# nanoporetech/taiyaki

Measured on AMD Instinct MI355X. Metric: signal-chunks/sec (T=4000) flip-flop train step, higher is better.
Workload: dtype f32; 1 GPU; configs[1]: mLstm_flipflop r9.4.1 DNA, chunk_len=4000 (T=800 blocks), 128 chunks/GPU, size 256, HIP flip-flop CRF loss + logZ, gradient maxima/clipping, AdamW; config_id=2, model=mLstm_flipflop, global_batch=128, chunk_len=4000, launch=hipGraph replay of forward+loss and of AdamW, eager backward, hw_queues=4, conv=gemm, lstm=miopen, batches=pre-assembled, cycled from HBM, parallelism=dp1 (reads sharded; one flat RCCL gradient all-reduce after backward)

## Files before the change

### taiyaki_amd/csrc/lstm_kernels.hip

```cpp
#include "dispatch.h"
#include "ff_common.h"
#include "lstm_bwd_layout.h"
#include "lstm_fwd_layout.h"
#include "rnn_common.h"

namespace tk {
namespace {

template <int U>
constexpr int threads_for() { return U == 48 ? 384 : U <= 32 ? 256 : 512; }
template <int H, int U>
constexpr int bwd_threads_for() { return U == 48 ? 2 * H : threads_for<U>(); }

template <int M>
__device__ __forceinline__ float xor_lane(float v) {
    static_assert(M == 1 || M == 2 || M == 4, "a partner inside the lane's group of 8");
    const int x = __float_as_int(v);
    if constexpr (M == 1) {
        return __int_as_float(__builtin_amdgcn_update_dpp(0, x, 0xB1, 0xF, 0xF, true));
    } else if constexpr (M == 2) {
        return __int_as_float(__builtin_amdgcn_update_dpp(0, x, 0x4E, 0xF, 0xF, true));
    } else {
        const int y = __builtin_amdgcn_update_dpp(0, x, 0x141, 0xF, 0xF, true);
        return __int_as_float(__builtin_amdgcn_update_dpp(0, y, 0x1B, 0xF, 0xF, true));
    }
}

template <int M, int RQ, int NA>
__device__ __forceinline__ void halve_rounds(float (&acc)[NA], int rq) {
    if constexpr (M < RQ) {
        constexpr int n = NA / (2 * M);
        const bool up = (rq & M) != 0;
#pragma unroll
        for (int a = 0; a < n; ++a) {
            const float send = up ? acc[a] : acc[a + n];
            const float keep = up ? acc[a + n] : acc[a];
            acc[a] = keep + xor_lane<M>(send);
        }
        halve_rounds<2 * M, RQ>(acc, rq);
    }
}

template <int H, int C, int U, bool VL, bool SAVE>
__device__ __forceinline__ void lstm_fwd_lanes_body(const float *__restrict__ gx, const float *__restrict__ whh, int T,
                                                    Cols cols, int reverse, int ngroups, float *__restrict__ y,
                                                    float *__restrict__ gates, float *__restrict__ cell, u64 *hbuf,
                                                    uint32_t *status, const int32_t *__restrict__ lengths) {
    constexpr int NT = threads_for<U>();
    const int N = cols.n, LD = cols.ld();
    constexpr int G = H / U;
    constexpr LstmFwdLanes FL(NT, H, U, C);
    constexpr int KP = FL.KP, KS = FL.KS, PR = FL.PR, CK = FL.CK;
    constexpr int NG = H * C / NT;
    static_assert(FL.ok() && KP == 8 && NG * NT == H * C && FL.gate_lane_xor(1) == 4 && FL.gate_lane_xor(2) == 2 &&
                      FL.gate_lane_xor(3) == 6,
                  "whole rows in 16-byte reads; the partial sums and the four gates of a column inside 8 lanes of a wave");
    constexpr int U4 = U / 4;
    constexpr int NQ = SAVE ? (6 * C * U4 + NT - 1) / NT : 1;
    static_assert(U % 4 == 0, "a row of the staging block is whole 16-byte chunks");
    __shared__ __attribute__((aligned(16))) float hs[2][H * C];
    __shared__ __attribute__((aligned(16))) float stg[SAVE ? 2 : 1][SAVE ? 6 * C * U : 4];
    __shared__ int give_up;

    int group, member;
    place(G, group, member);
    const int tid = threadIdx.x;
    const int j0 = member * U, n0 = group * C;
    const int u = tid / KP, kp = tid % KP;

    float w[4][KS];
#pragma unroll
    for (int g = 0; g < 4; ++g)
#pragma unroll
        for (int i = 0; i < KS; ++i) w[g][i] = whh[((size_t)g * H + j0 + u) * H + FL.k(kp, i)];
    settle(w);

    const int gate = FL.gate(kp), col = FL.col(kp, 0);
    const bool cell_lane = gate == 0;
    const int n = n0 + col;
    bool fetch[CK], valid[CK];
    float cst[CK], held[CK];
    int len[CK];
#pragma unroll
    for (int v = 0; v < CK; ++v) {
        fetch[v] = n + v < N;
        valid[v] = cell_lane && fetch[v];
        cst[v] = held[v] = 0.f;
        len[v] = 0;
        if constexpr (VL) len[v] = !valid[v] ? 0 : lengths ? lengths[n + v] : T;
    }

    for (int i = tid; i < H * C; i += NT) hs[0][i] = 0.f;
    if (tid == 0) give_up = 0;

    const size_t H4 = 4 * (size_t)H;
    float *rp[NQ];
    size_t rpitch[NQ];
    if constexpr (SAVE) {
#pragma unroll
        for (int i = 0; i < NQ; ++i) {
            const int q = tid + i * NT, row = q / U4, v = row / C, nn = n0 + row % C;
            const size_t w = v < 2 ? (size_t)H : H4;
            float *base = v == 0 ? y : v == 1 ? cell : gates + (size_t)(v - 2) * H;
            rpitch[i] = (size_t)LD * w;
            rp[i] = q < 6 * C * U4 && nn < N ? base + (size_t)nn * w + j0 + 4 * (q % U4) : nullptr;
        }
    }
    const float *gx0 = gx + (size_t)n * H4 + (size_t)gate * H + j0 + u;
    float gq[CK];
#pragma unroll
    for (int v = 0; v < CK; ++v) gq[v] = fetch[v] ? gx0[(size_t)(reverse ? T - 1 : 0) * LD * H4 + v * H4] : 0.f;
    __syncthreads();

    for (int s = 0; s < T; ++s) {
        const int t = reverse ? T - 1 - s : s;
        float *hb = hs[s & 1];
        settle(gq);
        if (s > 0) {
            const u64 *src = hbuf + ((size_t)((s - 1) & 1) * ngroups + group) * (H * C);
            float v[NG];
            if (!sweep<NG>(src, tid, NT, H * C, (unsigned)s, v, status)) give_up = 1;
#pragma unroll
            for (int q = 0; q < NG; ++q) {
                const int e = tid + q * NT;
                hb[FL.hs_index(e % H, e / H)] = v[q];
            }
            __syncthreads();
            if (give_up) return;
            const int tl = reverse ? t + 1 : t - 1;
            if constexpr (!SAVE) {
#pragma unroll
                for (int v = 0; v < CK; ++v)
                    if (valid[v]) y[((size_t)tl * LD + n + v) * H + j0 + u] = held[v];
            } else {
                rows_to_global<NQ>(stg[(s - 1) & 1], tid, NT, rp, rpitch, (size_t)tl);
            }
        }
        float gn[CK];
#pragma unroll
        for (int v = 0; v < CK; ++v)
            gn[v] = fetch[v] && s + 1 < T ? gx0[(size_t)(reverse ? t - 1 : t + 1) * LD * H4 + v * H4] : 0.f;
        asm volatile("" ::: "memory");

        float acc[4 * C];
#pragma unroll
        for (int a = 0; a < 4 * C; ++a) acc[a] = 0.f;
        constexpr int NR = KS / PR, AHEAD = 4;
        float hv[NR][PR * C];
#pragma unroll
        for (int j = 0; j < AHEAD; ++j) lds_row<PR * C>(hb + FL.chunk(kp, j), hv[j]);
#pragma unroll
        for (int j = 0; j < NR; ++j) {
            if (j + AHEAD < NR) lds_row<PR * C>(hb + FL.chunk(kp, j + AHEAD), hv[j + AHEAD]);
            __builtin_amdgcn_sched_barrier(0);
#pragma unroll
            for (int e = 0; e < PR; ++e)
#pragma unroll
                for (int g = 0; g < 4; ++g)
#pragma unroll
                    for (int c = 0; c < C; ++c)
                        acc[FL.flat(g, c)] = fmaf(w[g][PR * j + e], hv[j][e * C + c], acc[FL.flat(g, c)]);
        }
        halve_rounds<1, KP>(acc, kp);

        float ig[CK], fg[CK], gg[CK], og[CK];
#pragma unroll
        for (int v = 0; v < CK; ++v) {
            const float x = acc[v] + gq[v];
            float a;
            if (gate == 2)
                a = tanhf(x);
            else
                a = sigmoidf(x);
            ig[v] = a;
            gg[v] = xor_lane<2>(a);
            fg[v] = xor_lane<4>(a);
            og[v] = xor_lane<2>(fg[v]);
        }

        if (cell_lane) {
            float h[CK];
#pragma unroll
            for (int v = 0; v < CK; ++v) {
                cst[v] = fmaf(ig[v], gg[v], fg[v] * cst[v]);
                h[v] = og[v] * tanhf(cst[v]);
                if constexpr (VL) {
                    if (t >= len[v]) {
                        cst[v] = h[v] = 0.f;
                        if constexpr (SAVE) ig[v] = fg[v] = gg[v] = og[v] = 0.f;
                    }
                }
            }
            if (s + 1 < T) {
#pragma unroll
                for (int v = 0; v < CK; ++v)
                    store_granule(hbuf + ((size_t)(s & 1) * ngroups + group) * (H * C) + (col + v) * H + j0 + u,
                                  (unsigned)(s + 1), h[v]);
            }
#pragma unroll
            for (int v = 0; v < CK; ++v) {
                if constexpr (!SAVE) {
                    held[v] = h[v];
                } else {
                    float *sp = stg[s & 1] + (col + v) * U + u;
                    sp[0 * C * U] = h[v];
                    sp[1 * C * U] = cst[v];
                    sp[2 * C * U] = ig[v];
                    sp[3 * C * U] = fg[v];
                    sp[4 * C * U] = gg[v];
                    sp[5 * C * U] = og[v];
                }
            }
        }
#pragma unroll
        for (int v = 0; v < CK; ++v) gq[v] = gn[v];
    }
    if (T > 0) {
        const int tl = reverse ? 0 : T - 1;
        if constexpr (!SAVE) {
#pragma unroll
            for (int v = 0; v < CK; ++v)
                if (valid[v]) y[((size_t)tl * LD + n + v) * H + j0 + u] = held[v];
        } else {
            __syncthreads();
            rows_to_global<NQ>(stg[(T - 1) & 1], tid, NT, rp, rpitch, (size_t)tl);
        }
    }
}

template <int H, int C, int U, bool VL = false, bool SAVE = !VL>
__global__ __launch_bounds__(threads_for<U>(), 1) void lstm_fwd_kernel(const float *__restrict__ gx,
                                                                       const float *__restrict__ whh, int T, Cols cols,
                                                                       int reverse, int ngroups,
                                                                       float *__restrict__ y,
                                                                       float *__restrict__ gates,
                                                                       float *__restrict__ cell, u64 *hbuf,
                                                                       uint32_t *status,
                                                                       const int32_t *__restrict__ lengths) {
    if constexpr (lstm_fwd_lanes(H, U, C)) {
        lstm_fwd_lanes_body<H, C, U, VL, SAVE>(gx, whh, T, cols, reverse, ngroups, y, gates, cell, hbuf, status, lengths);
        return;
    }
    constexpr int NT = threads_for<U>();
    const int N = cols.n, LD = cols.ld();
    constexpr int G = H / U;
    constexpr int KP = NT / U;
    constexpr int KS = H / KP;
    constexpr int NG = (H * C + NT - 1) / NT;
    static_assert(KS >= 1 && KP <= 64 && C <= KP, "lane (u, kp) inside one wave; one cell lane per (u, column)");
    constexpr int U4 = U / 4;
    constexpr int NQ = SAVE ? (6 * C * U4 + NT - 1) / NT : 1;
    static_assert(U % 4 == 0, "a row of the staging block is whole 16-byte chunks");
    __shared__ __attribute__((aligned(16))) float hs[2][H * C];
    __shared__ __attribute__((aligned(16))) float stg[SAVE ? 2 : 1][SAVE ? 6 * C * U : 4];
    __shared__ int give_up;

    int group, member;
    place(G, group, member);
    const int tid = threadIdx.x;
    const int j0 = member * U, n0 = group * C;
    const int u = tid / KP, kp = tid % KP;

    float w[4][KS];
#pragma unroll
    for (int g = 0; g < 4; ++g)
#pragma unroll
        for (int i = 0; i < KS; ++i) w[g][i] = whh[((size_t)g * H + j0 + u) * H + i * KP + kp];
    settle(w);

    int col = 0;
#pragma unroll
    for (int m = 1, width = C; width > 1; m <<= 1, width >>= 1)
        if (kp & m) col += width / 2;
    const bool cell_lane = kp < C;
    const int n = n0 + col;
    const bool valid = cell_lane && n < N;
    float cst = 0.f;
    int len = 0;
    if constexpr (VL) len = !valid ? 0 : lengths ? lengths[n] : T;

    for (int i = tid; i < H * C; i += NT) hs[0][i] = 0.f;
    if (tid == 0) give_up = 0;

    const size_t H4 = 4 * (size_t)H;
    float *rp[NQ];
    size_t rpitch[NQ];
    if constexpr (SAVE) {
#pragma unroll
        for (int i = 0; i < NQ; ++i) {
            const int q = tid + i * NT, row = q / U4, v = row / C, nn = n0 + row % C;
            const size_t w = v < 2 ? (size_t)H : H4;
            float *base = v == 0 ? y : v == 1 ? cell : gates + (size_t)(v - 2) * H;
            rpitch[i] = (size_t)LD * w;
            rp[i] = q < 6 * C * U4 && nn < N ? base + (size_t)nn * w + j0 + 4 * (q % U4) : nullptr;
        }
    }
    float gq[4] = {0.f, 0.f, 0.f, 0.f};
    if (valid) {
        const float *p = gx + ((size_t)(reverse ? T - 1 : 0) * LD + n) * H4 + j0 + u;
#pragma unroll
        for (int g = 0; g < 4; ++g) gq[g] = p[(size_t)g * H];
    }
    float held = 0.f;
    __syncthreads();

    for (int s = 0; s < T; ++s) {
        const int t = reverse ? T - 1 - s : s;
        float *hb = hs[s & 1];
        settle(gq);
        if (s > 0) {
            const u64 *src = hbuf + ((size_t)((s - 1) & 1) * ngroups + group) * (H * C);
            float v[NG];
            if (!sweep<NG>(src, tid, NT, H * C, (unsigned)s, v, status)) give_up = 1;
#pragma unroll
            for (int q = 0; q < NG; ++q) {
                const int e = tid + q * NT;
                if (e < H * C) hb[(e % H) * C + e / H] = v[q];
            }
            __syncthreads();
            if (give_up) return;
            const int tl = reverse ? t + 1 : t - 1;
            if constexpr (!SAVE) {
                if (valid) y[((size_t)tl * LD + n) * H + j0 + u] = held;
            } else {
                rows_to_global<NQ>(stg[(s - 1) & 1], tid, NT, rp, rpitch, (size_t)tl);
            }
        }
        float gn[4] = {0.f, 0.f, 0.f, 0.f};
        if (valid && s + 1 < T) {
            const float *p = gx + ((size_t)(reverse ? t - 1 : t + 1) * LD + n) * H4 + j0 + u;
#pragma unroll
            for (int g = 0; g < 4; ++g) gn[g] = p[(size_t)g * H];
        }
        asm volatile("" ::: "memory");

        float acc[4][C];
#pragma unroll
        for (int g = 0; g < 4; ++g)
#pragma unroll
            for (int c = 0; c < C; ++c) acc[g][c] = 0.f;
#pragma unroll
        for (int i = 0; i < KS; ++i) {
            float hv[C];
            lds_row<C>(hb + (i * KP + kp) * C, hv);
#pragma unroll
            for (int g = 0; g < 4; ++g)
#pragma unroll
                for (int c = 0; c < C; ++c) acc[g][c] = fmaf(w[g][i], hv[c], acc[g][c]);
        }
#pragma unroll
        for (int m = 1; m < KP; m <<= 1) {
            const int half = C / (2 * m);
            const bool up = (kp & m) != 0;
#pragma unroll
            for (int g = 0; g < 4; ++g) {
                if (half == 0) acc[g][0] += __shfl_xor(acc[g][0], m);
#pragma unroll
                for (int c = 0; c < C / 2; ++c) {
                    if (c < half) {
                        const float send = up ? acc[g][c] : acc[g][c + half];
                        const float keep = up ? acc[g][c + half] : acc[g][c];
                        acc[g][c] = keep + __shfl_xor(send, m);
                    }
                }
            }
        }

        if (cell_lane) {
            float ig = sigmoidf(acc[0][0] + gq[0]), fg = sigmoidf(acc[1][0] + gq[1]);
            float gg = tanhf(acc[2][0] + gq[2]), og = sigmoidf(acc[3][0] + gq[3]);
            cst = fmaf(ig, gg, fg * cst);
            float h = og * tanhf(cst);
            if constexpr (VL) {
                if (t >= len) {
                    cst = h = 0.f;
                    if constexpr (SAVE) ig = fg = gg = og = 0.f;
                }
            }
            if (s + 1 < T)
                store_granule(hbuf + ((size_t)(s & 1) * ngroups + group) * (H * C) + col * H + j0 + u,
                              (unsigned)(s + 1), h);
            if constexpr (!SAVE) {
                held = h;
            } else {
                float *sp = stg[s & 1] + col * U + u;
                sp[0 * C * U] = h;
                sp[1 * C * U] = cst;
                sp[2 * C * U] = ig;
                sp[3 * C * U] = fg;
                sp[4 * C * U] = gg;
                sp[5 * C * U] = og;
            }
        }
#pragma unroll
        for (int g = 0; g < 4; ++g) gq[g] = gn[g];
    }
    if (T > 0) {
        const int tl = reverse ? 0 : T - 1;
        if constexpr (!SAVE) {
            if (valid) y[((size_t)tl * LD + n) * H + j0 + u] = held;
        } else {
            __syncthreads();
            rows_to_global<NQ>(stg[(T - 1) & 1], tid, NT, rp, rpitch, (size_t)tl);
        }
    }
}

#ifndef TK_RNN_VARLEN
template <int H, int C, int U, bool VL = false>
__global__ __launch_bounds__((bwd_threads_for<H, U>()), 1) void lstm_bwd_kernel(const float *__restrict__ whh,
                                                                       const float *__restrict__ gates,
                                                                       const float *__restrict__ cell,
                                                                       const float *__restrict__ dy, int T, Cols cols,
                                                                       int reverse, int ngroups,
                                                                       float *__restrict__ dgates, u64 *pbuf,
                                                                       uint32_t *status,
                                                                       const int32_t *__restrict__ lengths) {
    constexpr int NT = bwd_threads_for<H, U>();
    const int N = cols.n, LD = cols.ld();
    constexpr int G = H / U;
    constexpr bool STRIDED = U == 48;
    constexpr int RP = NT / H;
    constexpr int R = 4 * U / RP;
    constexpr LstmBwdBlock LB(NT, H, U, C);
    constexpr bool BLOCK = LB.KQ > 0;
    constexpr int KQ = BLOCK ? LB.KQ : 1, RQ = BLOCK ? LB.RQ : 1, RR = BLOCK ? LB.RR : 1, KEEP = BLOCK ? LB.KEEP : 1;
    constexpr int PAIRS = U * C;
    constexpr int PL = NT / PAIRS;
    constexpr int NP = (G + PL - 1) / PL;
    constexpr bool APART = BLOCK && NP > 1;
    static_assert(!APART || NP * PL == G, "every plane polls NP producers");
    static_assert(RP >= 1 && R >= 1 && PL >= 1 && PL * PAIRS == NT, "every lane polls; one cell lane per pair");
    static_assert(!STRIDED || (RP * H == NT && R * RP == 4 * U && U % RP == 0),
                  "a lane's rows keep their gate index at compile time");
    static_assert(!BLOCK || (LB.ok() && KQ * RR * NT == 4 * U * H && RQ <= 64 && (RQ & (RQ - 1)) == 0 &&
                             KEEP * NT == C * H && KQ * RR == R),
                  "every owned weight in one lane; the RQ partial sums inside one wave; one granule per held sum");
    __shared__ __attribute__((aligned(16))) float dgs[4 * U * C];
    __shared__ float gath[(APART ? G : PL) * PAIRS];
    __shared__ __attribute__((aligned(16))) float red[RP > 1 && !BLOCK ? RP * C * H : 1];
    __shared__ int give_up;

    int group, member;
    place(G, group, member);
    const int tid = threadIdx.x;
    const int j0 = member * U, n0 = group * C;

    const int k = tid % H, rp = tid / H;
    const int kb = tid / RQ, rq = tid % RQ;
    float w[R];
    if constexpr (BLOCK) {
#pragma unroll
        for (int j = 0; j < RR; ++j) {
            const int r = LB.row(rq, j);
#pragma unroll
            for (int q = 0; q < KQ; ++q) w[q * RR + j] = whh[((size_t)(r / U) * H + j0 + (r % U)) * H + KQ * kb + q];
        }
    } else if constexpr (STRIDED) {
        const float *wbase = whh + (size_t)(j0 + rp) * H + k;
#pragma unroll
        for (int i = 0; i < R; ++i) w[i] = wbase[(unsigned)((((i * RP) / U) * H + (i * RP) % U) * H)];
    } else {
#pragma unroll
        for (int i = 0; i < R; ++i) {
            const int r = rp * R + i;
            w[i] = whh[((size_t)(r / U) * H + j0 + (r % U)) * H + k];
        }
    }
    settle(w);

    const bool cell_lane = tid < PAIRS;
    const int pair = tid % PAIRS, plane = tid / PAIRS;
    const int cc = pair / U, u = pair % U;
    const int n = n0 + cc;
    const bool valid = cell_lane && n < N;
    float dc_next = 0.f, f_next = 0.f;
    int len = 0;
    if constexpr (VL) len = !valid ? 0 : lengths ? lengths[n] : T;
    if (tid == 0) give_up = 0;

    const size_t H4 = 4 * (size_t)H;
    float in[7] = {0.f, 0.f, 0.f, 0.f, 0.f, 0.f, 0.f};
    if (valid) {
        const int t = reverse ? 0 : T - 1;
        const size_t o = ((size_t)t * LD + n) * H + j0 + u;
        in[0] = dy[o];
        in[1] = cell[o];
        if (T > 1) in[2] = cell[((size_t)(reverse ? t + 1 : t - 1) * LD + n) * H + j0 + u];
        const float *gp = gates + ((size_t)t * LD + n) * H4 + j0 + u;
#pragma unroll
        for (int g = 0; g < 4; ++g) in[3 + g] = gp[(size_t)g * H];
    }
    float held[4] = {0.f, 0.f, 0.f, 0.f};
    __syncthreads();

    const u64 *mine = pbuf + (size_t)group * G * C * H + cc * H + j0 + u;
    const int a0 = LB.kept_first(rq), pub = (a0 % C) * H + KQ * kb + a0 / C;
    for (int s = 0; s < T; ++s) {
        const int tt = T - 1 - s;
        const int t = reverse ? T - 1 - tt : tt;
        const int tp = reverse ? t + 1 : t - 1;
        settle(in);
        float dhr = 0.f;
        if (s > 0) {
            float v[NP];
            const int nvalid = plane < G ? (G - plane + PL - 1) / PL : 0;
            const u64 *src = mine + (size_t)((s - 1) & 1) * ngroups * G * C * H;
            if (!sweep<NP>(src, plane * C * H, PL * C * H, G * C * H, (unsigned)s, v, status)) give_up = 1;
            if constexpr (APART) {
#pragma unroll
                for (int q = 0; q < NP; ++q) gath[(plane + q * PL) * PAIRS + pair] = v[q];
            } else {
                float sum = 0.f;
#pragma unroll
                for (int q = 0; q < NP; ++q)
                    if (q < nvalid) sum += v[q];
                gath[plane * PAIRS + pair] = sum;
            }
            __syncthreads();
            if (give_up) return;
            if (cell_lane) {
#pragma unroll
                for (int p = 0; p < (APART ? G : PL); ++p) dhr += gath[p * PAIRS + pair];
            }
            if (valid) {
                const int tl = reverse ? t - 1 : t + 1;
                float *dp = dgates + ((size_t)tl * LD + n) * H4 + j0 + u;
#pragma unroll
                for (int g = 0; g < 4; ++g) dp[(size_t)g * H] = held[g];
            }
        }
        float nx[7] = {0.f, 0.f, 0.f, 0.f, 0.f, 0.f, 0.f};
        if (valid && tt > 0) {
            const size_t o = ((size_t)tp * LD + n) * H + j0 + u;
            nx[0] = dy[o];
            nx[1] = in[2];
            if (tt > 1) nx[2] = cell[((size_t)(reverse ? tp + 1 : tp - 1) * LD + n) * H + j0 + u];
            const float *gp = gates + ((size_t)tp * LD + n) * H4 + j0 + u;
#pragma unroll
            for (int g = 0; g < 4; ++g) nx[3 + g] = gp[(size_t)g * H];
        }
        asm volatile("" ::: "memory");

        if (cell_lane) {
            const float ct = in[1];
            float cp = in[2];
            if constexpr (VL) {
                if (tp >= len) cp = 0.f;
            }
            const float ig = in[3], gg = in[5], og = in[6];
            float fg = in[4];
            const float dh = in[0] + dhr;
            const float tc = tanhf(ct);
            float dc = dh * og * (1.f - tc * tc) + dc_next * f_next;
            float di = dc * gg * ig * (1.f - ig);
            float df = dc * cp * fg * (1.f - fg);
            float dg = dc * ig * (1.f - gg * gg);
            float dout = dh * tc * og * (1.f - og);
            if constexpr (VL) {
                if (t >= len) dc = fg = di = df = dg = dout = 0.f;
            }
            dc_next = dc;
            f_next = fg;
            held[0] = di;
            held[1] = df;
            held[2] = dg;
            held[3] = dout;
            dgs[(0 * U + u) * C + cc] = valid ? di : 0.f;
            dgs[(1 * U + u) * C + cc] = valid ? df : 0.f;
            dgs[(2 * U + u) * C + cc] = valid ? dg : 0.f;
            dgs[(3 * U + u) * C + cc] = valid ? dout : 0.f;
        }
#pragma unroll
        for (int q = 0; q < 7; ++q) in[q] = nx[q];
        __syncthreads();
        if (s + 1 == T) break;

        if constexpr (BLOCK) {
            u64 *dst = pbuf + (((size_t)(s & 1) * ngroups + group) * G + member) * C * H;
            float acc[KQ * C];
#pragma unroll
            for (int a = 0; a < KQ * C; ++a) acc[a] = 0.f;
#pragma unroll
            for (int i = 0; i < RR / 2; ++i) {
                float d[2 * C];
                lds_row<2 * C>(dgs + (rq + RQ * i) * 2 * C, d);
#pragma unroll
                for (int e = 0; e < 2; ++e)
#pragma unroll
                    for (int q = 0; q < KQ; ++q)
#pragma unroll
                        for (int c = 0; c < C; ++c)
                            acc[q * C + c] = fmaf(w[q * RR + 2 * i + e], d[e * C + c], acc[q * C + c]);
            }
            halve_rounds<1, RQ>(acc, rq);
#pragma unroll
            for (int v = 0; v < KEEP; ++v) store_granule(dst + pub + v * H, (unsigned)(s + 1), acc[v]);
            continue;
        }
        float acc[C];
#pragma unroll
        for (int c = 0; c < C; ++c) acc[c] = 0.f;
#pragma unroll
        for (int i = 0; i < R; ++i) {
            float d[C];
            lds_row<C>(dgs + (STRIDED ? i * RP + rp : rp * R + i) * C, d);
#pragma unroll
            for (int c = 0; c < C; ++c) acc[c] = fmaf(w[i], d[c], acc[c]);
        }
        u64 *dst = pbuf + (((size_t)(s & 1) * ngroups + group) * G + member) * C * H;
        if constexpr (RP == 1) {
#pragma unroll
            for (int c = 0; c < C; ++c) store_granule(dst + c * H + k, (unsigned)(s + 1), acc[c]);
        } else {
#pragma unroll
            for (int c = 0; c < C; ++c) red[(rp * C + c) * H + k] = acc[c];
            __syncthreads();
            for (int e = tid; e < C * H; e += NT) {
                float v = 0.f;
#pragma unroll
                for (int q = 0; q < RP; ++q) v += red[q * C * H + e];
                store_granule(dst + e, (unsigned)(s + 1), v);
            }
        }
    }
    if (valid && T > 0) {
        const int tl = reverse ? T - 1 : 0;
        float *dp = dgates + ((size_t)tl * LD + n) * H4 + j0 + u;
#pragma unroll
        for (int g = 0; g < 4; ++g) dp[(size_t)g * H] = held[g];
    }
}

#endif

int g_lab_cols = 0;
int g_lab_units = 0;

int units48(size_t H) { return H == 192 || H == 384 ? 48 : 0; }

bool lstm_geometry(size_t N, size_t H, int cu_count, int *C_out, int *groups_out) {
    const int U48 = units48(H);
    if (!(U48 || H == 16 || H == 32 || H == 64 || H == 128 || H == 256) || N == 0 || cu_count <= 0) return false;
    const size_t G = H / (U48 ? U48 : 16);
    const int first = U48 ? 4 : 8, last = H == 384 ? 4 : 2 * first;
    for (int C = first; C <= last; C *= 2) {
        if (g_lab_cols != 0 && C != g_lab_cols) continue;
        const size_t groups = (N + C - 1) / C;
        if (groups * G <= (size_t)cu_count) {
            *C_out = C;
            *groups_out = (int)groups;
            return true;
        }
    }
    return false;
}

size_t ws_bytes(size_t H, int C, int groups, int U, bool backward) {
    return 2 * (size_t)groups * (backward ? H / U : 1) * C * H * sizeof(u64);
}

struct Plan {
    int U, C, groups;
    unsigned grid;
};

bool lstm_plan(size_t N, size_t H, int cu_count, Plan *p) {
    int C16 = 0, groups16 = 0;
    if (!lstm_geometry(N, H, cu_count, &C16, &groups16)) return false;
    if (const int U48 = units48(H)) {
        *p = Plan{U48, C16, groups16, (unsigned)(groups16 * (H / U48))};
        return true;
    }
    int U = g_lab_units != 0 ? g_lab_units : 64;
    if ((size_t)U > H) U = (int)H;
    if (U != 16 && U != 32 && U != 64) return false;
    p->U = U;
    p->C = C16 * 16 / U;
    p->groups = (int)((N + p->C - 1) / p->C);
    p->grid = (unsigned)(p->groups * (H / U));
    return true;
}

#define TK_LSTM_SWITCH(LAUNCH)                                                                                    \
    switch ((int)H * 100000 + p.U * 1000 + p.C) {                                                                 \
        LAUNCH(16, 16, 8) LAUNCH(16, 16, 16) LAUNCH(32, 16, 8) LAUNCH(32, 16, 16) LAUNCH(64, 16, 8)                \
        LAUNCH(64, 16, 16) LAUNCH(128, 16, 8) LAUNCH(128, 16, 16) LAUNCH(256, 16, 8) LAUNCH(256, 16, 16)          \
        LAUNCH(32, 32, 4) LAUNCH(32, 32, 8) LAUNCH(64, 32, 4) LAUNCH(64, 32, 8) LAUNCH(128, 32, 4)                 \
        LAUNCH(128, 32, 8) LAUNCH(256, 32, 4) LAUNCH(256, 32, 8)                                                  \
        LAUNCH(64, 64, 2) LAUNCH(64, 64, 4) LAUNCH(128, 64, 2) LAUNCH(128, 64, 4) LAUNCH(256, 64, 2)               \
        LAUNCH(256, 64, 4) LAUNCH(192, 48, 4) LAUNCH(192, 48, 8) LAUNCH(384, 48, 4)                               \
        default: return TK_ERR_UNSUPPORTED;                                                                       \
    }

template <bool VL, bool SAVE>
int launch_fwd(const Plan &p, size_t H, hipStream_t st, const float *gx, const float *whh, int T, Cols cols,
               int rev, float *y, float *gates, float *cell, u64 *ws, uint32_t *status, const int32_t *lengths) {
#define TK_LSTM_FWD(HH, UU, CC)                                                                                  \
    case HH * 100000 + UU * 1000 + CC:                                                                           \
        hipLaunchKernelGGL((lstm_fwd_kernel<HH, CC, UU, VL, SAVE>), dim3(p.grid), dim3(threads_for<UU>()), 0, st, gx,  \
                           whh, T, cols, rev, p.groups, y, gates, cell, ws, status, lengths);                    \
        break;
    TK_LSTM_SWITCH(TK_LSTM_FWD)
#undef TK_LSTM_FWD
    return hipGetLastError() == hipSuccess ? TK_OK : TK_ERR_LAUNCH;
}

#ifndef TK_RNN_VARLEN
template <bool VL>
int launch_bwd(const Plan &p, size_t H, hipStream_t st, const float *whh, const float *gates, const float *cell,
               const float *dy, int T, Cols cols, int rev, float *dg, u64 *ws, uint32_t *status,
               const int32_t *lengths) {
#define TK_LSTM_BWD(HH, UU, CC)                                                                                   \
    case HH * 100000 + UU * 1000 + CC:                                                                            \
        hipLaunchKernelGGL((lstm_bwd_kernel<HH, CC, UU, VL>), dim3(p.grid), dim3(bwd_threads_for<HH, UU>()), 0,   \
                           st, whh, gates, cell, dy, T, cols, rev, p.groups, dg, ws, status, lengths);            \
        break;
    TK_LSTM_SWITCH(TK_LSTM_BWD)
#undef TK_LSTM_BWD
    return hipGetLastError() == hipSuccess ? TK_OK : TK_ERR_LAUNCH;
}
#endif
#undef TK_LSTM_SWITCH

size_t lstm_slab(size_t N, size_t H, int cu_count) {
    int C = 0, groups = 0;
    const size_t S = widest_admitted([&](size_t n) { return lstm_geometry(n, H, cu_count, &C, &groups); });
    return N == 0 ? 0 : N < S ? N : S;
}

template <class Launch>
int checked(bool pointers_ok, size_t T, size_t N, size_t H, int cu_count, void *ws, size_t wsb, uint32_t *status,
            hipStream_t stream, bool backward, Launch launch) {
    if (!pointers_ok || !ws || !status || !aligned16(ws) || T > (size_t)INT32_MAX || N > (size_t)INT32_MAX)
        return TK_ERR_BAD_ARG;
#ifdef TK_RNN_WIDE
    const size_t S = lstm_slab(N, H, cu_count);
#else
    const size_t S = N;
#endif
    if (S == 0) return TK_ERR_UNSUPPORTED;
    for (size_t first = 0; first < N; first += S) {
        const size_t n = N - first < S ? N - first : S;
        Plan p;
        if (!lstm_plan(n, H, cu_count, &p)) return TK_ERR_UNSUPPORTED;
        const size_t need = ws_bytes(H, p.C, p.groups, p.U, backward);
        if (wsb < need) return TK_ERR_WORKSPACE;
        if (T == 0) continue;
        int rc = zero_ws(ws, need, stream);
        if (rc != TK_OK) return rc;
        rc = launch(p, first, make_cols(n, N));
        if (rc != TK_OK) return rc;
    }
    return TK_OK;
}

size_t train_workspace_bytes(size_t N, size_t H, int cu_count) {
    int C = 0, groups = 0;
    if (!lstm_geometry(N, H, cu_count, &C, &groups)) return 0;
    const int U48 = units48(H);
    return ws_bytes(H, C, groups, U48 ? U48 : 16, true);
}

template <bool VL, bool SAVE>
int forward(const float *gx, const float *whh, const int32_t *lengths, size_t T, size_t N, size_t H, int reverse,
            int cu_count, float *y, float *gates, float *cell, void *ws, size_t wsb, uint32_t *status,
            hipStream_t stream) {
    auto launch = [&](const Plan &p, size_t first, Cols cols) {
        return launch_fwd<VL, SAVE>(p, H, stream, at_column(gx, first, 4 * H), whh, (int)T, cols, reverse,
                                    at_column(y, first, H), at_column(gates, first, 4 * H), at_column(cell, first, H),
                                    static_cast<u64 *>(ws), status, at_column(lengths, first, 1));
    };
    return checked(gx && whh && y && (!SAVE || (gates && cell)), T, N, H, cu_count, ws, wsb, status, stream, false,
                   launch);
}

#ifndef TK_RNN_VARLEN
template <bool VL>
int backward(const float *whh, const float *gates, const float *cell, const float *dy, const int32_t *lengths,
             size_t T, size_t N, size_t H, int reverse, int cu_count, float *dgates, void *ws, size_t wsb,
             uint32_t *status, hipStream_t stream) {
    auto launch = [&](const Plan &p, size_t first, Cols cols) {
        return launch_bwd<VL>(p, H, stream, whh, at_column(gates, first, 4 * H), at_column(cell, first, H),
                              at_column(dy, first, H), (int)T, cols, reverse, at_column(dgates, first, 4 * H),
                              static_cast<u64 *>(ws), status, at_column(lengths, first, 1));
    };
    return checked(whh && gates && cell && dy && dgates, T, N, H, cu_count, ws, wsb, status, stream, true, launch);
}
#endif

}

#ifdef TK_RNN_VARLEN
size_t lstm_varlen_workspace_bytes(size_t N, size_t H, int cu_count) {
    Plan p;
    if (!lstm_plan(N, H, cu_count, &p)) return 0;
    return ws_bytes(H, p.C, p.groups, p.U, false);
}

int lstm_forward_varlen_dispatch(const float *gx, const float *whh, const int32_t *lengths, size_t T, size_t N,
                                 size_t H, int reverse, int cu_count, float *y, void *ws, size_t wsb,
                                 uint32_t *status, hipStream_t stream) {
    return forward<true, false>(gx, whh, lengths, T, N, H, reverse, cu_count, y, nullptr, nullptr, ws, wsb, status,
                                stream);
}
#elif defined(TK_RNN_VARLEN_TRAIN)
size_t lstm_varlen_train_workspace_bytes(size_t N, size_t H, int cu_count) {
    return train_workspace_bytes(N, H, cu_count);
}

int lstm_forward_varlen_save_dispatch(const float *gx, const float *whh, const int32_t *lengths, size_t T, size_t N,
                                      size_t H, int reverse, int cu_count, float *y, float *gates, float *cell,
                                      void *ws, size_t wsb, uint32_t *status, hipStream_t stream) {
    return forward<true, true>(gx, whh, lengths, T, N, H, reverse, cu_count, y, gates, cell, ws, wsb, status, stream);
}

int lstm_backward_varlen_dispatch(const float *whh, const float *gates, const float *cell, const float *dy,
                                  const int32_t *lengths, size_t T, size_t N, size_t H, int reverse, int cu_count,
                                  float *dgates, void *ws, size_t wsb, uint32_t *status, hipStream_t stream) {
    return backward<true>(whh, gates, cell, dy, lengths, T, N, H, reverse, cu_count, dgates, ws, wsb, status, stream);
}
#elif defined(TK_RNN_WIDE)
size_t lstm_wide_slab(size_t N, size_t H, int cu_count) { return lstm_slab(N, H, cu_count); }

size_t lstm_wide_workspace_bytes(size_t N, size_t H, int cu_count) {
    return train_workspace_bytes(lstm_slab(N, H, cu_count), H, cu_count);
}

int lstm_forward_wide_dispatch(const float *gx, const float *whh, const int32_t *lengths, size_t T, size_t N,
                               size_t H, int reverse, int cu_count, float *y, float *gates, float *cell, void *ws,
                               size_t wsb, uint32_t *status, hipStream_t stream) {
    if (!gates != !cell) return TK_ERR_BAD_ARG;
    return gates ? forward<true, true>(gx, whh, lengths, T, N, H, reverse, cu_count, y, gates, cell, ws, wsb, status,
                                       stream)
                 : forward<true, false>(gx, whh, lengths, T, N, H, reverse, cu_count, y, nullptr, nullptr, ws, wsb,
                                        status, stream);
}

int lstm_backward_wide_dispatch(const float *whh, const float *gates, const float *cell, const float *dy,
                                const int32_t *lengths, size_t T, size_t N, size_t H, int reverse, int cu_count,
                                float *dgates, void *ws, size_t wsb, uint32_t *status, hipStream_t stream) {
    return backward<true>(whh, gates, cell, dy, lengths, T, N, H, reverse, cu_count, dgates, ws, wsb, status, stream);
}
#else
size_t lstm_workspace_bytes(size_t N, size_t H, int cu_count) { return train_workspace_bytes(N, H, cu_count); }

int lstm_forward_dispatch(const float *gx, const float *whh, size_t T, size_t N, size_t H, int reverse,
                          int cu_count, float *y, float *gates, float *cell, void *ws, size_t wsb,
                          uint32_t *status, hipStream_t stream) {
    return forward<false, true>(gx, whh, nullptr, T, N, H, reverse, cu_count, y, gates, cell, ws, wsb, status, stream);
}

int lstm_backward_dispatch(const float *whh, const float *gates, const float *cell, const float *dy, size_t T,
                           size_t N, size_t H, int reverse, int cu_count, float *dgates, void *ws, size_t wsb,
                           uint32_t *status, hipStream_t stream) {
    return backward<false>(whh, gates, cell, dy, nullptr, T, N, H, reverse, cu_count, dgates, ws, wsb, status, stream);
}

#ifdef TK_LAB
void lstm_lab_cols(int cols) { g_lab_cols = cols; }
void lstm_lab_units(int units) { g_lab_units = units; }

bool lstm_lab_geometry(size_t N, size_t H, int cu_count, size_t *out) {
    int C16 = 0, groups16 = 0;
    Plan p;
    if (!lstm_geometry(N, H, cu_count, &C16, &groups16) || !lstm_plan(N, H, cu_count, &p)) return false;
    const size_t v[8] = {(size_t)C16, (size_t)groups16, (size_t)p.U, (size_t)p.C, (size_t)p.groups, p.grid,
                         ws_bytes(H, p.C, p.groups, p.U, false), ws_bytes(H, p.C, p.groups, p.U, true)};
    for (int i = 0; i < 8; ++i) out[i] = v[i];
    return true;
}
#endif
#endif

}
```

### taiyaki_amd/csrc/rnn_common.h

```cpp
#pragma once
#include <hip/hip_runtime.h>
#include <math.h>
#include <stdint.h>

#include "../../include/taiyaki_amd_flipflop.h"

namespace tk {
namespace {

constexpr uint64_t kSpinTicks = 200000000ull;

struct Cols {
    int n;
#ifdef TK_RNN_WIDE
    int pitch;
    __host__ __device__ int ld() const { return pitch; }
#else
    __host__ __device__ int ld() const { return n; }
#endif
};

inline Cols make_cols(size_t n, size_t ld) {
#ifdef TK_RNN_WIDE
    return Cols{(int)n, (int)ld};
#else
    return Cols{(int)n};
#endif
}

template <class P>
P *at_column(P *p, size_t first, size_t width) {
    return p ? p + first * width : p;
}

template <class Admits>
size_t widest_admitted(Admits admits) {
    size_t lo = 1, hi = (size_t)INT32_MAX;
    if (!admits(lo)) return 0;
    if (admits(hi)) return hi;
    while (hi - lo > 1) {
        const size_t mid = lo + (hi - lo) / 2;
        (admits(mid) ? lo : hi) = mid;
    }
    return lo;
}

typedef unsigned long long u64;
typedef __attribute__((address_space(1))) u64 gu64;
typedef __attribute__((address_space(1))) uint32_t gu32;

__device__ __forceinline__ void store_granule(u64 *g, unsigned tag, float v) {
    __hip_atomic_store((gu64 *)g, ((u64)tag << 32) | __float_as_uint(v), __ATOMIC_RELAXED,
                       __HIP_MEMORY_SCOPE_AGENT);
}

template <int NG>
__device__ __forceinline__ bool sweep(const u64 *g, int e0, int stride, int end, unsigned tag, float (&v)[NG],
                                      uint32_t *status) {
    const uint64_t start = __builtin_amdgcn_s_memrealtime();
    for (unsigned spins = 0;; ++spins) {
        bool ok = true;
#pragma unroll
        for (int q = 0; q < NG; ++q) {
            const int e = e0 + q * stride;
            const bool in = e < end;
            const u64 x = __hip_atomic_load((gu64 *)(g + (in ? e : 0)), __ATOMIC_RELAXED, __HIP_MEMORY_SCOPE_AGENT);
            v[q] = __uint_as_float((unsigned)x);
            ok &= !in || (unsigned)(x >> 32) == tag;
        }
        if (__all(ok)) return true;
        if ((spins & 31) == 31) {
            const uint32_t st = __hip_atomic_load((gu32 *)status, __ATOMIC_RELAXED, __HIP_MEMORY_SCOPE_AGENT);
            if ((st & TK_STATUS_RNN_TIMEOUT) || __builtin_amdgcn_s_memrealtime() - start > kSpinTicks) {
                __hip_atomic_fetch_or((gu32 *)status, TK_STATUS_RNN_TIMEOUT, __ATOMIC_RELAXED,
                                      __HIP_MEMORY_SCOPE_AGENT);
                return false;
            }
        }
        __builtin_amdgcn_s_sleep(1);
    }
}

__device__ __forceinline__ void place(int G, int &group, int &member) {
    const int b = blockIdx.x, nb = gridDim.x;
    int L = b;
    if (nb % 8 == 0 && (nb / 8) % G == 0) L = (b % 8) * (nb / 8) + b / 8;
    group = L / G;
    member = L % G;
}

template <int M>
__device__ __forceinline__ void settle(float (&v)[M]) {
#pragma unroll
    for (int i = 0; i < M; ++i) asm volatile("" : "+v"(v[i]));
}
template <int M, int K>
__device__ __forceinline__ void settle(float (&v)[M][K]) {
#pragma unroll
    for (int i = 0; i < M; ++i) settle(v[i]);
}

__device__ __forceinline__ float sigmoidf(float x) { return 1.f / (1.f + expf(-x)); }

template <int C>
__device__ __forceinline__ void lds_row(const float *p, float (&v)[C]) {
    if constexpr (C % 4 == 0) {
#pragma unroll
        for (int c4 = 0; c4 < C / 4; ++c4) {
            const float4 q = reinterpret_cast<const float4 *>(p)[c4];
            v[4 * c4 + 0] = q.x;
            v[4 * c4 + 1] = q.y;
            v[4 * c4 + 2] = q.z;
            v[4 * c4 + 3] = q.w;
        }
    } else if constexpr (C == 2) {
        const float2 q = *reinterpret_cast<const float2 *>(p);
        v[0] = q.x;
        v[1] = q.y;
    } else {
#pragma unroll
        for (int c = 0; c < C; ++c) v[c] = p[c];
    }
}

typedef float row_chunk __attribute__((ext_vector_type(4), aligned(4)));

template <int NQ>
__device__ __forceinline__ void rows_to_global(const float *blk, int tid, int nt, float *const (&dst)[NQ],
                                               const size_t (&pitch)[NQ], size_t t) {
#pragma unroll
    for (int i = 0; i < NQ; ++i) {
        if (!dst[i]) continue;
        const float4 v = reinterpret_cast<const float4 *>(blk)[tid + i * nt];
        *reinterpret_cast<row_chunk *>(dst[i] + t * pitch[i]) = row_chunk{v.x, v.y, v.z, v.w};
    }
}

__global__ void zero_u64x2_kernel(uint4 *p, size_t n) {
    for (size_t i = (size_t)blockIdx.x * blockDim.x + threadIdx.x; i < n; i += (size_t)gridDim.x * blockDim.x)
        p[i] = make_uint4(0u, 0u, 0u, 0u);
}

int zero_ws(void *ws, size_t bytes, hipStream_t stream) {
    const size_t n = bytes / 16;
    const unsigned blocks = (unsigned)((n + 255) / 256 < 1024 ? (n + 255) / 256 : 1024);
    hipLaunchKernelGGL(zero_u64x2_kernel, dim3(blocks), dim3(256), 0, stream, static_cast<uint4 *>(ws), n);
    return hipGetLastError() == hipSuccess ? TK_OK : TK_ERR_LAUNCH;
}

}
}
```

Baseline: 5586 chunks/s.

## Strength-reduce LSTM step addressing and overlap saved-state stores with recurrent matvec

Replaces per-step global index arithmetic in the persistent LSTM forward and backward kernels with pointers in the global address space that advance by a fixed stride each step, pinned with asm barriers. In the forward SAVE path, the staged h/c/gate rows are read from LDS before the recurrent FMA loop and written to global memory inside its first iteration, so the stores overlap compute instead of sitting on the serial step path. The give-up check is moved after the matvec. In backward, the tanh and (1-x) gate-derivative factors are computed at the top of the step with FP contraction turned off. This adds register pressure and brittle asm ordering constraints, and a timeout now exits one step's compute later.

```diff
diff --git a/taiyaki_amd/csrc/lstm_kernels.hip b/taiyaki_amd/csrc/lstm_kernels.hip
--- a/taiyaki_amd/csrc/lstm_kernels.hip
+++ b/taiyaki_amd/csrc/lstm_kernels.hip
@@ -94,28 +94,60 @@
     if (tid == 0) give_up = 0;
 
     const size_t H4 = 4 * (size_t)H;
-    float *rp[NQ];
-    size_t rpitch[NQ];
+    const ptrdiff_t dir = reverse ? -1 : 1, t0 = reverse ? T - 1 : 0;
+    gfloat *rp[NQ];
+    ptrdiff_t rstep[NQ];
+    bool rok[NQ];
     if constexpr (SAVE) {
 #pragma unroll
         for (int i = 0; i < NQ; ++i) {
             const int q = tid + i * NT, row = q / U4, v = row / C, nn = n0 + row % C;
             const size_t w = v < 2 ? (size_t)H : H4;
             float *base = v == 0 ? y : v == 1 ? cell : gates + (size_t)(v - 2) * H;
-            rpitch[i] = (size_t)LD * w;
-            rp[i] = q < 6 * C * U4 && nn < N ? base + (size_t)nn * w + j0 + 4 * (q % U4) : nullptr;
-        }
-    }
+            rstep[i] = dir * (ptrdiff_t)((size_t)LD * w);
+            rok[i] = q < 6 * C * U4 && nn < N;
+            rp[i] = (gfloat *)base + (size_t)nn * w + j0 + 4 * (q % U4) + (t0 - 2 * dir) * (ptrdiff_t)((size_t)LD * w);
+        }
+    }
+    const float4 *stg4 = reinterpret_cast<const float4 *>(&stg[0][0]);
+    gfloat *yp = (gfloat *)y + ((t0 - 2 * dir) * LD + n) * (ptrdiff_t)H + j0 + u;
+    const ptrdiff_t ystep = dir * (ptrdiff_t)LD * H;
     const float *gx0 = gx + (size_t)n * H4 + (size_t)gate * H + j0 + u;
+    const ptrdiff_t gstep = dir * (ptrdiff_t)((size_t)LD * H4);
+    gcfloat *gxp = (gcfloat *)gx0 + t0 * (ptrdiff_t)((size_t)LD * H4);
     float gq[CK];
 #pragma unroll
-    for (int v = 0; v < CK; ++v) gq[v] = fetch[v] ? gx0[(size_t)(reverse ? T - 1 : 0) * LD * H4 + v * H4] : 0.f;
+    for (int v = 0; v < CK; ++v) gq[v] = fetch[v] ? gxp[v * H4] : 0.f;
+    u64 *const pub0 = hbuf + (size_t)group * (H * C) + col * H + j0 + u;
+    const size_t pubpitch = (size_t)ngroups * (H * C);
     __syncthreads();
 
     for (int s = 0; s < T; ++s) {
         const int t = reverse ? T - 1 - s : s;
         float *hb = hs[s & 1];
         settle(gq);
+        gxp += gstep;
+        settle_ptr(gxp);
+        if constexpr (SAVE) {
+#pragma unroll
+            for (int i = 0; i < NQ; ++i) {
+                rp[i] += rstep[i];
+                settle_ptr(rp[i]);
+            }
+        } else {
+            yp += ystep;
+            settle_ptr(yp);
+        }
+        gu64 *pub = (gu64 *)pub0 + (s & 1) * pubpitch;
+        settle_ptr(pub);
+        int blk[NQ];
+        if constexpr (SAVE) {
+#pragma unroll
+            for (int i = 0; i < NQ; ++i) {
+                blk[i] = rok[i] ? ((s - 1) & 1) * (6 * C * U4) + tid + i * NT : 0;
+                asm volatile("" : "+v"(blk[i]));
+            }
+        }
         if (s > 0) {
             const u64 *src = hbuf + ((size_t)((s - 1) & 1) * ngroups + group) * (H * C);
             float v[NG];
@@ -126,20 +158,15 @@
                 hb[FL.hs_index(e % H, e / H)] = v[q];
             }
             __syncthreads();
-            if (give_up) return;
-            const int tl = reverse ? t + 1 : t - 1;
             if constexpr (!SAVE) {
 #pragma unroll
                 for (int v = 0; v < CK; ++v)
-                    if (valid[v]) y[((size_t)tl * LD + n + v) * H + j0 + u] = held[v];
-            } else {
-                rows_to_global<NQ>(stg[(s - 1) & 1], tid, NT, rp, rpitch, (size_t)tl);
+                    if (valid[v]) yp[v * H] = held[v];
             }
         }
         float gn[CK];
 #pragma unroll
-        for (int v = 0; v < CK; ++v)
-            gn[v] = fetch[v] && s + 1 < T ? gx0[(size_t)(reverse ? t - 1 : t + 1) * LD * H4 + v * H4] : 0.f;
+        for (int v = 0; v < CK; ++v) gn[v] = fetch[v] && s + 1 < T ? gxp[v * H4] : 0.f;
         asm volatile("" ::: "memory");
 
         float acc[4 * C];
@@ -149,6 +176,12 @@
         float hv[NR][PR * C];
 #pragma unroll
         for (int j = 0; j < AHEAD; ++j) lds_row<PR * C>(hb + FL.chunk(kp, j), hv[j]);
+        const int gu = give_up;
+        float4 out[NQ];
+        if constexpr (SAVE) {
+#pragma unroll
+            for (int i = 0; i < NQ; ++i) out[i] = stg4[blk[i]];
+        }
 #pragma unroll
         for (int j = 0; j < NR; ++j) {
             if (j + AHEAD < NR) lds_row<PR * C>(hb + FL.chunk(kp, j + AHEAD), hv[j + AHEAD]);
@@ -160,8 +193,20 @@
 #pragma unroll
                     for (int c = 0; c < C; ++c)
                         acc[FL.flat(g, c)] = fmaf(w[g][PR * j + e], hv[j][e * C + c], acc[FL.flat(g, c)]);
+            if constexpr (SAVE) {
+                if (j == 0) {
+#pragma unroll
+                    for (int i = 0; i < NQ; ++i) {
+#pragma unroll
+                        for (int a = 0; a < 4 * C; ++a) asm volatile("" : "+v"(out[i].x) : "v"(acc[a]));
+                        if (rok[i] && s > 0) *(grow_chunk *)rp[i] = row_chunk{out[i].x, out[i].y, out[i].z, out[i].w};
+                    }
+                    asm volatile("" ::: "memory");
+                }
+            }
         }
         halve_rounds<1, KP>(acc, kp);
+        if (gu) return;
 
         float ig[CK], fg[CK], gg[CK], og[CK];
 #pragma unroll
@@ -193,9 +238,7 @@
             }
             if (s + 1 < T) {
 #pragma unroll
-                for (int v = 0; v < CK; ++v)
-                    store_granule(hbuf + ((size_t)(s & 1) * ngroups + group) * (H * C) + (col + v) * H + j0 + u,
-                                  (unsigned)(s + 1), h[v]);
+                for (int v = 0; v < CK; ++v) store_granule((u64 *)(pub + v * H), (unsigned)(s + 1), h[v]);
             }
 #pragma unroll
             for (int v = 0; v < CK; ++v) {
@@ -216,14 +259,18 @@
         for (int v = 0; v < CK; ++v) gq[v] = gn[v];
     }
     if (T > 0) {
-        const int tl = reverse ? 0 : T - 1;
         if constexpr (!SAVE) {
 #pragma unroll
             for (int v = 0; v < CK; ++v)
-                if (valid[v]) y[((size_t)tl * LD + n + v) * H + j0 + u] = held[v];
+                if (valid[v]) yp[ystep + v * H] = held[v];
         } else {
             __syncthreads();
-            rows_to_global<NQ>(stg[(T - 1) & 1], tid, NT, rp, rpitch, (size_t)tl);
+#pragma unroll
+            for (int i = 0; i < NQ; ++i) {
+                if (!rok[i]) continue;
+                const float4 o = stg4[((T - 1) & 1) * (6 * C * U4) + tid + i * NT];
+                *(grow_chunk *)(rp[i] + rstep[i]) = row_chunk{o.x, o.y, o.z, o.w};
+            }
         }
     }
 }
@@ -492,6 +539,11 @@
         for (int g = 0; g < 4; ++g) in[3 + g] = gp[(size_t)g * H];
     }
     float held[4] = {0.f, 0.f, 0.f, 0.f};
+    const ptrdiff_t step1 = (reverse ? 1 : -1) * (ptrdiff_t)LD * H, step4 = 4 * step1;
+    const ptrdiff_t row0 = ((ptrdiff_t)(reverse ? 0 : T - 1) * LD + n) * H;
+    gcfloat *dyp = (gcfloat *)dy + row0 + j0 + u, *cnp = (gcfloat *)cell + row0 + step1 + j0 + u;
+    gcfloat *gp = (gcfloat *)gates + 4 * row0 + j0 + u;
+    gfloat *dgp = (gfloat *)dgates + 4 * row0 - 2 * step4 + j0 + u;
     __syncthreads();
 
     const u64 *mine = pbuf + (size_t)group * G * C * H + cc * H + j0 + u;
@@ -501,7 +553,29 @@
         const int t = reverse ? T - 1 - tt : tt;
         const int tp = reverse ? t + 1 : t - 1;
         settle(in);
+        float fac[6] = {0.f, 0.f, 0.f, 0.f, 0.f, 0.f};
+        if (cell_lane) {
+#pragma clang fp contract(off)
+            const float tc = tanhf(in[1]);
+            fac[0] = fmaf(-tc, tc, 1.f);
+            fac[1] = 1.f - in[3];
+            fac[2] = 1.f - in[4];
+            const float g2 = in[5] * in[5];
+            fac[3] = 1.f - g2;
+            fac[4] = 1.f - in[6];
+            fac[5] = tc;
+        }
+        settle(fac);
+        dyp += step1;
+        cnp += step1;
+        gp += step4;
+        dgp += step4;
+        settle_ptr(dyp);
+        settle_ptr(cnp);
+        settle_ptr(gp);
+        settle_ptr(dgp);
         float dhr = 0.f;
+        int gu = 0;
         if (s > 0) {
             float v[NP];
             const int nvalid = plane < G ? (G - plane + PL - 1) / PL : 0;
@@ -518,32 +592,28 @@
                 gath[plane * PAIRS + pair] = sum;
             }
             __syncthreads();
-            if (give_up) return;
+            gu = give_up;
             if (cell_lane) {
 #pragma unroll
                 for (int p = 0; p < (APART ? G : PL); ++p) dhr += gath[p * PAIRS + pair];
             }
             if (valid) {
-                const int tl = reverse ? t - 1 : t + 1;
-                float *dp = dgates + ((size_t)tl * LD + n) * H4 + j0 + u;
-#pragma unroll
-                for (int g = 0; g < 4; ++g) dp[(size_t)g * H] = held[g];
+#pragma unroll
+                for (int g = 0; g < 4; ++g) dgp[(size_t)g * H] = held[g];
             }
         }
         float nx[7] = {0.f, 0.f, 0.f, 0.f, 0.f, 0.f, 0.f};
         if (valid && tt > 0) {
-            const size_t o = ((size_t)tp * LD + n) * H + j0 + u;
-            nx[0] = dy[o];
+            nx[0] = *dyp;
             nx[1] = in[2];
-            if (tt > 1) nx[2] = cell[((size_t)(reverse ? tp + 1 : tp - 1) * LD + n) * H + j0 + u];
-            const float *gp = gates + ((size_t)tp * LD + n) * H4 + j0 + u;
+            if (tt > 1) nx[2] = *cnp;
 #pragma unroll
             for (int g = 0; g < 4; ++g) nx[3 + g] = gp[(size_t)g * H];
         }
         asm volatile("" ::: "memory");
 
         if (cell_lane) {
-            const float ct = in[1];
+#pragma clang fp contract(off)
             float cp = in[2];
             if constexpr (VL) {
                 if (tp >= len) cp = 0.f;
@@ -551,12 +621,12 @@
             const float ig = in[3], gg = in[5], og = in[6];
             float fg = in[4];
             const float dh = in[0] + dhr;
-            const float tc = tanhf(ct);
-            float dc = dh * og * (1.f - tc * tc) + dc_next * f_next;
-            float di = dc * gg * ig * (1.f - ig);
-            float df = dc * cp * fg * (1.f - fg);
-            float dg = dc * ig * (1.f - gg * gg);
-            float dout = dh * tc * og * (1.f - og);
+            const float tc = fac[5];
+            float dc = fmaf(dc_next, f_next, dh * og * fac[0]);
+            float di = dc * gg * ig * fac[1];
+            float df = dc * cp * fg * fac[2];
+            float dg = dc * ig * fac[3];
+            float dout = dh * tc * og * fac[4];
             if constexpr (VL) {
                 if (t >= len) dc = fg = di = df = dg = dout = 0.f;
             }
@@ -573,6 +643,7 @@
         }
 #pragma unroll
         for (int q = 0; q < 7; ++q) in[q] = nx[q];
+        if (gu) return;
         __syncthreads();
         if (s + 1 == T) break;
 
diff --git a/taiyaki_amd/csrc/rnn_common.h b/taiyaki_amd/csrc/rnn_common.h
--- a/taiyaki_amd/csrc/rnn_common.h
+++ b/taiyaki_amd/csrc/rnn_common.h
@@ -100,6 +100,14 @@
     for (int i = 0; i < M; ++i) settle(v[i]);
 }
 
+typedef __attribute__((address_space(1))) float gfloat;
+typedef __attribute__((address_space(1))) const float gcfloat;
+
+template <class P>
+__device__ __forceinline__ void settle_ptr(P *&p) {
+    asm volatile("" : "+v"(p));
+}
+
 __device__ __forceinline__ float sigmoidf(float x) { return 1.f / (1.f + expf(-x)); }
 
 template <int C>
@@ -124,6 +132,7 @@
 }
 
 typedef float row_chunk __attribute__((ext_vector_type(4), aligned(4)));
+typedef __attribute__((address_space(1))) row_chunk grow_chunk;
 
 template <int NQ>
 __device__ __forceinline__ void rows_to_global(const float *blk, int tid, int nt, float *const (&dst)[NQ],
```

After: 5821 chunks/s, median of 6. +4.2%, better.
